# kenoogl/CubeZ

Hardware: AMD Instinct MI355X
Metric: MLUPS (lattice updates/s), 512^3 FP32 Jacobi per GPU (higher is better)
Workload: dtype f32

## Files before the change

### cubez_amd/csrc/cz_k_jac3.h

```cpp

template <int V, int TB, int UNIT, int MED>
__global__ void __launch_bounds__(TB, 1)
jac3_k(const REAL* __restrict__ U, const REAL* __restrict__ B, REAL* __restrict__ W, Coef c, Geom2 g, double* partials,
       const int* __restrict__ skip, Fin2 fin) {
  if (skip != nullptr && *skip != 0) return;
  extern __shared__ __attribute__((aligned(16))) char smem[];
  const int t = threadIdx.x;
  const int R = g.R;
  constexpr int LV = TB;
  const DeepLds<V> lds = deep_lds<V, LV, 3>(smem, R);
  const int LU = lds.LU;
  Vec<V>* ldsU = lds.U;
  Vec<V>* ldsF = lds.F;
  double* wsum = lds.wsum;

  const PassItem it = pass_item<V>(g);
  const int ja = it.ja, jb = it.jb;

  double acc1 = 0.0, acc2 = 0.0, acc3 = 0.0;
  const typename std::conditional<MED != 0, MediumDiv, HoistedDiv>::type dv{fastdiv_init(c.dd)};

  if (it.work) {
    const long long e2_0 = it.fb - 2 * (long long)R;
    const size_t PB = (size_t)g.PSB;
    const RowView<V> rv = row_view<V>(g, it);
    const int x = t;
    const long long f = e2_0 + x;
    const unsigned bo = rv.off_of(f);
    const VecMask mk = vec_mask<V>(g, it, f);
    const unsigned inbox = mk.rows ? mk.bits : 0u;
    const unsigned own = (x >= 2 * R && x < LV - 2 * R && mk.rows && mk.kown) ? mk.bits : 0u;
    const bool wave2 = __builtin_amdgcn_ballot_w64(x >= R && x < LV - R) != 0ull;
    const bool wave3 = __builtin_amdgcn_ballot_w64(own != 0) != 0ull;
    const OuterRow h = outer_row<V, TB>(rv, LV, it.fb - 3 * (long long)R, f);
    const char* Ub = reinterpret_cast<const char*>(U);
    const char* Bb = reinterpret_cast<const char*>(B);
    char* Wb = reinterpret_cast<char*>(W);

    const int q0 = ja - 2;
    Vec<V> uA, uB, bA, bB, hx;
    {
      const Vec<V> t2 = ld16<V>(Ub + (size_t)rv.pl(q0 - 1) * PB, rv.lim(bo, rv.pl(q0 - 1)));
      const Vec<V> t1 = ld16<V>(Ub + (size_t)rv.pl(q0) * PB, rv.lim(bo, rv.pl(q0)));
      const Vec<V> h1 = ld16<V>(Ub + (size_t)rv.pl(q0) * PB, rv.lim(h.bo, rv.pl(q0)));
      uA = ld16<V>(Ub + (size_t)rv.pl(q0 + 1) * PB, rv.lim(bo, rv.pl(q0 + 1)));
      bA = ld16<V>(Bb + (size_t)rv.pl(q0) * PB, rv.lim(bo, rv.pl(q0)));
      ldsU[(size_t)((q0 - 1) & 1) * LU + R + x] = t2;
      ldsU[(size_t)(q0 & 1) * LU + R + x] = t1;
      if (h.has) ldsU[(size_t)(q0 & 1) * LU + h.hl] = h1;
    }
    Vec<V> bq1 = zerov<V>(), bq2 = zerov<V>();
    __syncthreads();

    const int x_first = __builtin_amdgcn_readfirstlane(x), x_last = __builtin_amdgcn_readlane(x, 63);
    auto stage = [&](const Vec<V>* cur, const Vec<V>* prv, const Vec<V>& nxt, const Vec<V>& bb, unsigned msk, unsigned cnt,
                     double& acc) __attribute__((always_inline)) -> Vec<V> {
      const Vec<V> pc = lds_ld<V>(cur + x);
      const Vec<V> im = lds_ld<V>(cur + x - R);
      const Vec<V> ip = lds_ld<V>(cur + x + R);
      const Vec<V> pm = lds_ld<V>(prv + x);
      const REAL elo = reinterpret_cast<const REAL*>(cur)[(long long)x_first * V - 1];
      const REAL ehi = reinterpret_cast<const REAL*>(cur)[(long long)(x_last + 1) * V];
      const REAL kl = lane_shr1(elo, pc.v[V - 1]);
      const REAL kr = lane_shl1(ehi, pc.v[0]);
      return relax_vec<V, UNIT>(pc, im, ip, pm, nxt, kl, kr, bb, c, dv, msk, cnt, acc);
    };

    const char* uN = Ub;
    const char* bN = Bb;
    char* wN = Wb;
    auto step = [&](auto inner, const int q, Vec<V>& uc, Vec<V>& un, Vec<V>& b1, Vec<V>& bn) __attribute__((always_inline)) {
      constexpr bool INNER = decltype(inner)::value;
      if constexpr (INNER) {
        hx = ld16<V>(uN, h.bo);
        un = ld16<V>(uN + PB, bo);
        bn = ld16<V>(bN, bo);
      } else {
        const int qu = rv.pl(q + 2 <= jb + 3 ? q + 2 : jb + 3), qb = rv.pl(q + 1 <= jb + 2 ? q + 1 : jb + 2);
        hx = ld16<V>(Ub + (size_t)rv.pl(q + 1) * PB, rv.lim(h.bo, rv.pl(q + 1)));
        un = ld16<V>(Ub + (size_t)qu * PB, rv.lim(bo, qu));
        bn = ld16<V>(Bb + (size_t)qb * PB, rv.lim(bo, qb));
      }
      const int p1 = q, p2 = q - 1, p3 = q - 2;
      auto upd = [&](int p) -> unsigned { return (INNER || (p >= g.jj0 && p <= g.jj1)) ? inbox : 0u; };
      auto cnt = [&](int p) -> unsigned { return (INNER || (p >= ja && p <= jb)) ? own : 0u; };
      const Vec<V>* cU = ldsU + (size_t)(p1 & 1) * LU + R;
      const Vec<V>* pU = ldsU + (size_t)((p1 - 1) & 1) * LU + R;
      Vec<V>* F1 = ldsF;
      Vec<V>* F2 = ldsF + (size_t)2 * LV;
      const Vec<V> v1 = stage(cU, pU, uc, b1, upd(p1), cnt(p1), acc1);
      Vec<V> v2 = v1;
      if (wave2) v2 = stage(F1 + (size_t)(p2 & 1) * LV, F1 + (size_t)((p2 - 1) & 1) * LV, v1, bq1, upd(p2), cnt(p2), acc2);
      if ((INNER || p3 >= ja) && wave3) {
        const Vec<V> o = stage(F2 + (size_t)(p3 & 1) * LV, F2 + (size_t)((p3 - 1) & 1) * LV, v2, bq2, own, own, acc3);
        store_owned<V>(INNER ? wN : Wb + (size_t)p3 * PB, bo, own, o);
      }
      F1[(size_t)(p1 & 1) * LV + x] = v1;
      F2[(size_t)(p2 & 1) * LV + x] = v2;
      Vec<V>* nU = ldsU + (size_t)((p1 + 1) & 1) * LU;
      nU[R + x] = uc;
      if (h.has) nU[h.hl] = hx;
      bq2 = bq1, bq1 = b1;
      if constexpr (INNER) uN += PB, bN += PB, wN += PB;
      __syncthreads();
    };
    const int qi = jb < g.jlast - 3 ? jb : g.jlast - 3;
    int q = q0;
#pragma nounroll
    for (int phase = 0; phase < 2; phase++) {
      const int qg = phase == 0 ? ja + 1 : jb + 2;
      for (;;) {
        step(std::false_type{}, q, uA, uB, bA, bB);
        if (++q > qg) break;
        step(std::false_type{}, q, uB, uA, bB, bA);
        if (++q > qg) break;
      }
      if (phase == 0) {
        uN = Ub + (size_t)(q + 1) * PB, bN = Bb + (size_t)(q + 1) * PB, wN = Wb + (size_t)(q - 2) * PB;
        for (; q + 1 <= qi; q += 2) {
          step(std::true_type{}, q, uA, uB, bA, bB);
          step(std::true_type{}, q + 1, uB, uA, bB, bA);
        }
      }
    }
  }

  const double acc[3] = {acc1, acc2, acc3};
  pass_epilogue<TB, 3>(acc, partials, fin, wsum);
}
```

Before: 995,900.

## Rotate B registers via 4x unroll and defer halo load past first stage

Unrolls the inner Jacobi loop by four so the B-field history (b1/b2/b3) rotates through register renaming instead of copying values each step. Moves the halo-row global load after the first stencil stage, prefetching one plane ahead, and skips it for waves with no halo lanes. Uses empty asm constraints to keep base pointers scalar, offsets in vector registers, and to pin where the first stage's result is materialised. This trades more code size and register pressure, and may leave remainder iterations on the slower outer path.

```diff
diff --git a/cubez_amd/csrc/cz_k_jac3.h b/cubez_amd/csrc/cz_k_jac3.h
--- a/cubez_amd/csrc/cz_k_jac3.h
+++ b/cubez_amd/csrc/cz_k_jac3.h
@@ -1,3 +1,22 @@
+
+template <class T>
+__device__ __forceinline__ T* uniform_global(T* p) {
+  auto g = (__attribute__((address_space(1))) T*)p;
+  asm("" : "+s"(g));
+  return (T*)g;
+}
+
+__device__ __forceinline__ unsigned lane_offset(unsigned o) {
+  asm("" : "+v"(o));
+  return o;
+}
+
+template <int V>
+__device__ __forceinline__ void complete_here(Vec<V>& x) {
+  static_assert(V == 2 || V == 4, "one constraint per component");
+  if constexpr (V == 4) asm volatile("" : "+v"(x.v[0]), "+v"(x.v[1]), "+v"(x.v[2]), "+v"(x.v[3]));
+  else asm volatile("" : "+v"(x.v[0]), "+v"(x.v[1]));
+}
 
 template <int V, int TB, int UNIT, int MED>
 __global__ void __launch_bounds__(TB, 1)
@@ -26,23 +45,28 @@
     const RowView<V> rv = row_view<V>(g, it);
     const int x = t;
     const long long f = e2_0 + x;
-    const unsigned bo = rv.off_of(f);
+    unsigned bo = rv.off_of(f);
     const VecMask mk = vec_mask<V>(g, it, f);
     const unsigned inbox = mk.rows ? mk.bits : 0u;
     const unsigned own = (x >= 2 * R && x < LV - 2 * R && mk.rows && mk.kown) ? mk.bits : 0u;
     const bool wave2 = __builtin_amdgcn_ballot_w64(x >= R && x < LV - R) != 0ull;
     const bool wave3 = __builtin_amdgcn_ballot_w64(own != 0) != 0ull;
-    const OuterRow h = outer_row<V, TB>(rv, LV, it.fb - 3 * (long long)R, f);
+    OuterRow h = outer_row<V, TB>(rv, LV, it.fb - 3 * (long long)R, f);
+    const bool waveh = __builtin_amdgcn_ballot_w64(h.has) != 0ull;
     const char* Ub = reinterpret_cast<const char*>(U);
     const char* Bb = reinterpret_cast<const char*>(B);
     char* Wb = reinterpret_cast<char*>(W);
 
     const int q0 = ja - 2;
-    Vec<V> uA, uB, bA, bB, hx;
+    Vec<V> uA, uB, bA, bB, hx = zerov<V>();
     {
       const Vec<V> t2 = ld16<V>(Ub + (size_t)rv.pl(q0 - 1) * PB, rv.lim(bo, rv.pl(q0 - 1)));
       const Vec<V> t1 = ld16<V>(Ub + (size_t)rv.pl(q0) * PB, rv.lim(bo, rv.pl(q0)));
-      const Vec<V> h1 = ld16<V>(Ub + (size_t)rv.pl(q0) * PB, rv.lim(h.bo, rv.pl(q0)));
+      Vec<V> h1 = zerov<V>();
+      if (waveh) {
+        h1 = ld16<V>(Ub + (size_t)rv.pl(q0) * PB, rv.lim(h.bo, rv.pl(q0)));
+        hx = ld16<V>(Ub + (size_t)rv.pl(q0 + 1) * PB, rv.lim(h.bo, rv.pl(q0 + 1)));
+      }
       uA = ld16<V>(Ub + (size_t)rv.pl(q0 + 1) * PB, rv.lim(bo, rv.pl(q0 + 1)));
       bA = ld16<V>(Bb + (size_t)rv.pl(q0) * PB, rv.lim(bo, rv.pl(q0)));
       ldsU[(size_t)((q0 - 1) & 1) * LU + R + x] = t2;
@@ -69,18 +93,21 @@
     const char* uN = Ub;
     const char* bN = Bb;
     char* wN = Wb;
-    auto step = [&](auto inner, const int q, Vec<V>& uc, Vec<V>& un, Vec<V>& b1, Vec<V>& bn) __attribute__((always_inline)) {
+    auto step = [&](auto inner, const int q, Vec<V>& uc, Vec<V>& un, Vec<V>& b1, Vec<V>& bn, Vec<V>& b2, Vec<V>& b3) __attribute__((always_inline)) {
       constexpr bool INNER = decltype(inner)::value;
+      const char *up, *bp;
+      unsigned uo, bo1, ho;
       if constexpr (INNER) {
-        hx = ld16<V>(uN, h.bo);
-        un = ld16<V>(uN + PB, bo);
-        bn = ld16<V>(bN, bo);
+        uN = uniform_global(uN), bN = uniform_global(bN), wN = uniform_global(wN);
+        bo = lane_offset(bo), h.bo = lane_offset(h.bo);
+        up = uN, bp = bN, uo = bo, bo1 = bo, ho = h.bo;
       } else {
         const int qu = rv.pl(q + 2 <= jb + 3 ? q + 2 : jb + 3), qb = rv.pl(q + 1 <= jb + 2 ? q + 1 : jb + 2);
-        hx = ld16<V>(Ub + (size_t)rv.pl(q + 1) * PB, rv.lim(h.bo, rv.pl(q + 1)));
-        un = ld16<V>(Ub + (size_t)qu * PB, rv.lim(bo, qu));
-        bn = ld16<V>(Bb + (size_t)qb * PB, rv.lim(bo, qb));
+        up = Ub + (size_t)qu * PB, bp = Bb + (size_t)qb * PB;
+        uo = rv.lim(bo, qu), bo1 = rv.lim(bo, qb), ho = rv.lim(h.bo, qu);
       }
+      un = ld16<V>(up, uo);
+      bn = ld16<V>(bp, bo1);
       const int p1 = q, p2 = q - 1, p3 = q - 2;
       auto upd = [&](int p) -> unsigned { return (INNER || (p >= g.jj0 && p <= g.jj1)) ? inbox : 0u; };
       auto cnt = [&](int p) -> unsigned { return (INNER || (p >= ja && p <= jb)) ? own : 0u; };
@@ -88,19 +115,23 @@
       const Vec<V>* pU = ldsU + (size_t)((p1 - 1) & 1) * LU + R;
       Vec<V>* F1 = ldsF;
       Vec<V>* F2 = ldsF + (size_t)2 * LV;
-      const Vec<V> v1 = stage(cU, pU, uc, b1, upd(p1), cnt(p1), acc1);
+      Vec<V> v1 = stage(cU, pU, uc, b1, upd(p1), cnt(p1), acc1);
+      complete_here<V>(v1);
+      if (waveh) {
+        if (h.has) ldsU[(size_t)((p1 + 1) & 1) * LU + h.hl] = hx;
+        hx = ld16<V>(up, ho);
+      }
       Vec<V> v2 = v1;
-      if (wave2) v2 = stage(F1 + (size_t)(p2 & 1) * LV, F1 + (size_t)((p2 - 1) & 1) * LV, v1, bq1, upd(p2), cnt(p2), acc2);
+      if (wave2) v2 = stage(F1 + (size_t)(p2 & 1) * LV, F1 + (size_t)((p2 - 1) & 1) * LV, v1, b2, upd(p2), cnt(p2), acc2);
       if ((INNER || p3 >= ja) && wave3) {
-        const Vec<V> o = stage(F2 + (size_t)(p3 & 1) * LV, F2 + (size_t)((p3 - 1) & 1) * LV, v2, bq2, own, own, acc3);
+        const Vec<V> o = stage(F2 + (size_t)(p3 & 1) * LV, F2 + (size_t)((p3 - 1) & 1) * LV, v2, b3, own, own, acc3);
         store_owned<V>(INNER ? wN : Wb + (size_t)p3 * PB, bo, own, o);
       }
       F1[(size_t)(p1 & 1) * LV + x] = v1;
       F2[(size_t)(p2 & 1) * LV + x] = v2;
       Vec<V>* nU = ldsU + (size_t)((p1 + 1) & 1) * LU;
       nU[R + x] = uc;
-      if (h.has) nU[h.hl] = hx;
-      bq2 = bq1, bq1 = b1;
+      if constexpr (!INNER) b3 = b2, b2 = b1;
       if constexpr (INNER) uN += PB, bN += PB, wN += PB;
       __syncthreads();
     };
@@ -110,16 +141,18 @@
     for (int phase = 0; phase < 2; phase++) {
       const int qg = phase == 0 ? ja + 1 : jb + 2;
       for (;;) {
-        step(std::false_type{}, q, uA, uB, bA, bB);
+        step(std::false_type{}, q, uA, uB, bA, bB, bq1, bq2);
         if (++q > qg) break;
-        step(std::false_type{}, q, uB, uA, bB, bA);
+        step(std::false_type{}, q, uB, uA, bB, bA, bq1, bq2);
         if (++q > qg) break;
       }
       if (phase == 0) {
-        uN = Ub + (size_t)(q + 1) * PB, bN = Bb + (size_t)(q + 1) * PB, wN = Wb + (size_t)(q - 2) * PB;
-        for (; q + 1 <= qi; q += 2) {
-          step(std::true_type{}, q, uA, uB, bA, bB);
-          step(std::true_type{}, q + 1, uB, uA, bB, bA);
+        uN = Ub + (size_t)(q + 2) * PB, bN = Bb + (size_t)(q + 1) * PB, wN = Wb + (size_t)(q - 2) * PB;
+        for (; q + 3 <= qi; q += 4) {
+          step(std::true_type{}, q, uA, uB, bA, bB, bq1, bq2);
+          step(std::true_type{}, q + 1, uB, uA, bB, bq2, bA, bq1);
+          step(std::true_type{}, q + 2, uA, uB, bq2, bq1, bB, bA);
+          step(std::true_type{}, q + 3, uB, uA, bq1, bA, bq2, bB);
         }
       }
     }
```

Result: faster. 1.039 million, median of 6 (+4.4%).
